# ChengZhang-98/lqer

Measured on AMD Instinct MI355X. Metric: W4A8+rank-r Linear GEMM TFLOPS-equiv, higher is better.
Workload: dtype bf16; 1 GPU; LqerLinear 4096x4096 rank32 W4A8-MXINT16 M=2048 (BASELINE configs[1]); rank=32, formats=x MXINT8/16, W MXINT4/16, A_out,B_out as x, y fp16, weights=one Linear

## Files before the change

include/lqer_hip.h:

```cpp
#ifndef LQER_HIP_H
#define LQER_HIP_H

#include <stddef.h>
#include <stdint.h>

#ifdef __cplusplus
extern "C" {
#endif

#define LQER_ABI_VERSION 14

#define LQER_OK 0
#define LQER_E_INVALID (-1)
#define LQER_E_UNSUPPORTED (-2)
#define LQER_E_LAUNCH (-3)
#define LQER_E_WORKSPACE (-4)

#define LQER_F32 0
#define LQER_F16 1
#define LQER_BF16 2

#define LQER_Q_PASSTHROUGH 0
#define LQER_Q_MXINT 1
#define LQER_Q_PASSTHROUGH_F16 2
// ... 16 lines not shown
  int32_t width;
  int32_t block;
  int32_t exp_width;
  int32_t exp_bias;
} lqer_qfmt_t;

typedef struct lqer_linear_desc {
  int32_t in_features;
  int32_t out_features;
  int32_t rank;
  int32_t has_bias;
  lqer_qfmt_t x_fmt;
  lqer_qfmt_t w_fmt;
  lqer_qfmt_t b_fmt;
  lqer_qfmt_t a_out_fmt;
  lqer_qfmt_t b_out_fmt;
  int32_t tuning;
} lqer_linear_desc_t;

#define LQER_TUNE_TILE_ROWS_128 0x1
#define LQER_TUNE_TILE_ROWS_64 0x2
#define LQER_TUNE_I8_ROWS_128 0x4
#define LQER_TUNE_I8_ROWS_256 0x8
#define LQER_TUNE_AMAX_ATOMIC 0x40000
#define LQER_TUNE_AMAX_PARTS 0x80000
#define LQER_TUNE_AMAX_XCH_MISS 0x100000
#define LQER_TUNE_ACT8_SPLIT 0x200000
#define LQER_TUNE_ACT8_FUSED 0x400000
#define LQER_TUNE_ACT16_SPLIT 0x800000
#define LQER_TUNE_ACT16_FUSED 0x1000000
#define LQER_TUNE_AMAX_NO_MRX 0x4000000
#define LQER_TUNE_BOUT_IN_PROLOGUE 0x2000000
#define LQER_TUNE_W_EXP_TABLE 0x8000000
#define LQER_TUNE_DECODE_NO_POLL 0x10000

typedef struct lqer_linear_sizes {
  size_t w_packed;
  size_t a_t;
  size_t b_t;
  size_t bias_q;
  size_t workspace;
} lqer_linear_sizes_t;

int lqer_version(void);
const char* lqer_last_error(void);
size_t lqer_sizeof_qfmt(void);
size_t lqer_sizeof_linear_desc(void);
size_t lqer_sizeof_linear_sizes(void);
size_t lqer_sizeof_group_member(void);

int64_t lqer_padded_k(int64_t K);
int64_t lqer_padded_n(int64_t N);
int64_t lqer_padded_m(int64_t M);
int64_t lqer_padded_r(int64_t r);


int lqer_quantize_mxint(const void* x, int dtype, int64_t rows, int64_t cols, int64_t ld,
                        const lqer_qfmt_t* fmt, float* deq_f32, int8_t* codes, int8_t* exps,
                        void* stream);

int lqer_quantize_mxint_tiles(const void* x, int dtype, int64_t batches, int64_t rows, int64_t cols, const lqer_qfmt_t* fmt,
                              int64_t tile_rows, int64_t tile_cols, float* deq_f32, float* amax_scratch, void* stream);

int lqer_quantize_act_mxint(const void* x, int dtype, int64_t M, int64_t K, int64_t ldx,
                            const lqer_qfmt_t* fmt, void* xq_bf16, void* stream);

// ... 193 lines not shown
```

lqer_amd/_lib.py:

```python
from __future__ import annotations

import ctypes as C
import os
import subprocess
from typing import Optional

_HERE = os.path.dirname(os.path.abspath(__file__))
LIB_PATH = os.environ.get("LQER_AMD_LIB") or os.path.join(_HERE, "liblqer_hip.so")
BUILD_SCRIPT = os.path.join(_HERE, "csrc", "build.sh")

ABI_VERSION = 14
F32, F16, BF16 = 0, 1, 2
Q_PASSTHROUGH, Q_MXINT, Q_PASSTHROUGH_F16, Q_MXINT_I8, Q_INT, Q_MINIFLOAT = 0, 1, 2, 3, 4, 5
K_ALIGN, M_ALIGN, N_ALIGN, R_ALIGN = 64, 256, 256, 16
ROUTE_SMALLM, ROUTE_TILE128, ROUTE_TILE256, ROUTE_I8 = 0, 1, 2, 3
TUNE_TILE_ROWS_128, TUNE_TILE_ROWS_64, TUNE_DECODE_NO_POLL = 0x1, 0x2, 0x10000
TUNE_I8_ROWS_128, TUNE_I8_ROWS_256, TUNE_AMAX_ATOMIC, TUNE_AMAX_PARTS = 0x4, 0x8, 0x40000, 0x80000
TUNE_ACT16_SPLIT, TUNE_ACT16_FUSED = 0x800000, 0x1000000
TUNE_ACT8_SPLIT, TUNE_ACT8_FUSED = 0x200000, 0x400000
TUNE_AMAX_NO_MRX = 0x4000000
TUNE_BOUT_IN_PROLOGUE = 0x2000000
TUNE_W_EXP_TABLE = 0x8000000
TUNE_AMAX_XCH_MISS = 0x100000


class QFmt(C.Structure):
    _fields_ = [("kind", C.c_int32), ("width", C.c_int32), ("block", C.c_int32), ("exp_width", C.c_int32), ("exp_bias", C.c_int32)]


class LinearDesc(C.Structure):
    _fields_ = [
        ("in_features", C.c_int32),
        ("out_features", C.c_int32),
        ("rank", C.c_int32),
        ("has_bias", C.c_int32),
        ("x_fmt", QFmt),
        ("w_fmt", QFmt),
        ("b_fmt", QFmt),
        ("a_out_fmt", QFmt),
        ("b_out_fmt", QFmt),
        ("tuning", C.c_int32),
    ]


class GroupMember(C.Structure):
    _fields_ = [("desc", C.POINTER(LinearDesc)), ("w_packed", C.c_void_p), ("b_t", C.c_void_p), ("b_limbs", C.c_int32),
                ("bias_q", C.c_void_p), ("y", C.c_void_p), ("ldy", C.c_int64)]


class LinearSizes(C.Structure):
    _fields_ = [("w_packed", C.c_size_t), ("a_t", C.c_size_t), ("b_t", C.c_size_t), ("bias_q", C.c_size_t), ("workspace", C.c_size_t)]


_vp, _i, _i64, _sz = C.c_void_p, C.c_int, C.c_int64, C.c_size_t
# ... 130 lines not shown
```

lqer_amd/csrc/gemm_plan.h:

```cpp
#pragma once
#include "common.h"

namespace lqer {

enum AmaxTravel {
  AMAX_NONE = 0,
  AMAX_CELLS,
  AMAX_PARTS,
  AMAX_XCH,
  AMAX_MRX,
};

struct GemmPlan {
  int err, launch_err;
  char msg[256];
  bool empty;

  int bout;
  int bout_L, bout_nblk;
  int route;
  int tile_rows;
  int tiles_m, tiles_n;
  unsigned grid;

  bool lowrank;
  bool f16x;
  bool staged, defer;
  bool w_twos, w_mf;
  bool i8_shift, i8_codes;
  int mt;

  AmaxTravel amax;
  size_t need;
  size_t zero_bytes;
  size_t prep_zero_bytes;
  struct {
    bool lds;
    int rg, nks;
    unsigned grid;
    int tiles_n32, seg_tiles;
    int nseg;
  } pre;
};

GemmPlan plan_gemm(const GemmArgs& shape, bool lowrank, bool i8_image, int dtype, int cus);

int device_cus();

int gemm_launch(const GemmPlan& p, GemmArgs g, int dtype, void* scratch, size_t scratch_bytes, bool amax_zeroed, hipStream_t st);
int launch_amax(const GemmPlan& p, const GemmArgs& g, bool amax_zeroed, hipStream_t st);
int tile128_launch(const GemmPlan& p, const GemmArgs& g, int dtype, hipStream_t st);
int m256_launch(const GemmPlan& p, const GemmArgs& g, int dtype, hipStream_t st);
int i8_launch(const GemmPlan& p, const GemmArgs& g, int dtype, hipStream_t st);
int smallm_launch(const GemmPlan& p, const GemmArgs& g, int dtype, hipStream_t st);

}
```

lqer_amd/csrc/gemm_plan.hip:

```cpp
#include <stdarg.h>
#include <stdio.h>

#include "gemm_plan.h"

namespace lqer {

namespace {

constexpr int64_t PLAN_CUS = 256;

int refuse(GemmPlan& p, bool at_launch, int code, const char* fmt, ...) {
  if (p.err || p.launch_err) return code;
  (at_launch ? p.launch_err : p.err) = code;
  va_list ap;
  va_start(ap, fmt);
  vsnprintf(p.msg, sizeof(p.msg), fmt, ap);
  va_end(ap);
  return code;
}

int64_t rounds(int64_t tiles) { return (tiles + PLAN_CUS - 1) / PLAN_CUS; }

int i8_tile_rows(const GemmArgs& g) {
  if (g.tuning & LQER_TUNE_I8_ROWS_128) return 128;
// ... 130 lines not shown
    if (p.amax == AMAX_CELLS || p.amax == AMAX_PARTS) plan_prepass(p, g);
  }

  if (i8_image && !i8_ok)
    refuse(p, true, LQER_E_UNSUPPORTED,
           "linear_gemm: LQER_Q_MXINT_I8 is not served for M=%d here (lqer_gemm_route != LQER_ROUTE_I8): call with LQER_Q_MXINT", g.M);
  switch (p.route) {
    case LQER_ROUTE_I8:
      p.tiles_m = (g.M + p.tile_rows - 1) / p.tile_rows, p.tiles_n = g.Np / BN;
      p.grid = (unsigned)(p.tiles_m * p.tiles_n < PLAN_CUS ? p.tiles_m * p.tiles_n : PLAN_CUS);
      p.i8_codes = g.w_i8codes, p.i8_shift = g.i8_shift;
      break;
    case LQER_ROUTE_SMALLM:
      p.grid = (unsigned)(g.Np / 16);
      p.mt = g.M > 48 ? 4 : (g.M + 15) / 16;
      break;
    case LQER_ROUTE_TILE256:
      p.tiles_m = (g.M + 255) / 256, p.tiles_n = g.Np / BN;
      p.grid = (unsigned)(p.tiles_m * p.tiles_n);
      break;
    default:
      p.tiles_m = (g.M + p.tile_rows - 1) / p.tile_rows, p.tiles_n = g.Np / BN;
      p.grid = (unsigned)(p.tiles_m * p.tiles_n);
      p.w_twos = g.w_twos, p.w_mf = g.w_mf;
      if (p.f16x && (p.w_mf || p.bout == 3))
        refuse(p, true, LQER_E_UNSUPPORTED,
               "linear_gemm: minifloat weights and B_out have no fp16 main loop (pass-through fp16 activations take the limb route)");
      else if (p.f16x && p.w_twos)
        refuse(p, true, LQER_E_UNSUPPORTED,
               "linear_gemm: integer weights have no fp16 main loop (pass-through fp16 activations take the limb route)");
      p.staged = lowrank && (p.w_twos || p.w_mf || g.rp * g.b_limbs > LQER_STAGE_MIN);
      p.defer = p.bout == 1 && !nibbles128 && p.tile_rows == 128 && !(g.tuning & LQER_TUNE_BOUT_IN_PROLOGUE) && g.Kp / BK >= 16 &&
                g.bout.kind == LQER_Q_MXINT && g.bout.mmax <= 4194304.0f && g.bout.mneg <= 4194304.0f && g.bout.tiny >= 1e-8f;
      break;
  }
  return p;
}

}
```

lqer_amd/csrc/gemm_w4a8.hip:

```cpp
#include <type_traits>
#include <utility>

#include "gemm_plan.h"
#include "gemm_tile.h"

namespace lqer {

#ifndef LQER_DEPTH
#define LQER_DEPTH 3
#endif
constexpr int DEPTH = LQER_DEPTH;
constexpr int NSLOT = DEPTH + 1;
constexpr int R_SLOT = (BN / 16) * LQER_PANEL_BYTES;
constexpr int OFF_A = 0;
constexpr int a_slot_bytes(int mt) { return 32 * mt * BK * 2; }
constexpr int gemm_lds_bytes(int mt) { return NSLOT * a_slot_bytes(mt) + NSLOT * R_SLOT; }

template <int OFF>
__device__ __forceinline__ bf16x8 lds_read128(uint32_t addr) {
  bf16x8 v;
  asm volatile("ds_read_b128 %0, %1 offset:%2" : "=v"(v) : "v"(addr), "i"(OFF));
  return v;
}
__device__ __forceinline__ u32x4 lds_read128u(uint32_t addr) {
  u32x4 v;
  asm volatile("ds_read_b128 %0, %1" : "=v"(v) : "v"(addr));
  return v;
}
__device__ __forceinline__ uint32_t lds_read32_512(uint32_t addr) {
  uint32_t v;
  asm volatile("ds_read_b32 %0, %1 offset:512" : "=v"(v) : "v"(addr));
  return v;
}
__device__ __forceinline__ u32x2 lds_read64(uint32_t addr) {
  u32x2 v;
  asm volatile("ds_read_b64 %0, %1" : "=v"(v) : "v"(addr));
  return v;
}
__device__ __forceinline__ int lds_read_i8_512(uint32_t addr) {
  int v;
  asm volatile("ds_read_i8 %0, %1 offset:512" : "=v"(v) : "v"(addr));
  return v;
}
__device__ __forceinline__ void lds_write128(uint32_t addr, u32x4 v) {
  asm volatile("ds_write_b128 %0, %1" ::"v"(addr), "v"(v) : "memory");
}
__device__ __forceinline__ void lds_wait(bf16x8& a, bf16x8& b, bf16x8& c, bf16x8& d) {
  asm volatile("s_waitcnt lgkmcnt(0)" : "+v"(a), "+v"(b), "+v"(c), "+v"(d));
}
__device__ __forceinline__ void lds_wait(bf16x8& a, bf16x8& b) {
  asm volatile("s_waitcnt lgkmcnt(0)" : "+v"(a), "+v"(b));
}
__device__ __forceinline__ void lds_wait(u32x2& a, int& b) {
  asm volatile("s_waitcnt lgkmcnt(0)" : "+v"(a), "+v"(b));
}

#ifdef LQER_STAMPS
#define LQER_LOAD_BARRIER ""
#else
#define LQER_LOAD_BARRIER "\n\ts_barrier"
#endif
#if defined(LQER_STAMPS) || defined(LQER_CLOCKPROBE)
__device__ unsigned long long* g_stamp_buf = nullptr;
#endif
#ifdef LQER_STAMPS
#define STAMP(i)                                                                        \
  do {                                                                                  \
    unsigned long long t_;                                                              \
    __builtin_amdgcn_sched_barrier(0);                                                  \
    asm volatile("s_memtime %0\n\ts_waitcnt lgkmcnt(0)" : "=s"(t_)::"memory");         \
    __builtin_amdgcn_sched_barrier(0);                                                  \
    st_sum[i] += t_ - st_prev;                                                          \
    st_prev = t_;                                                                       \
  } while (0)
#else
#define STAMP(i)
#endif

template <int DT, bool LOWRANK, int BOUT, bool STAGED = false, int MT = 4, bool WTWOS = false, bool DEFER = false, bool WMF = false>
__global__ __launch_bounds__(512) void k_lqer_gemm(GemmArgs g) {
  static_assert(MT == 4 || MT == 2, "128- or 64-row tiles");
  static_assert(!DEFER || (LOWRANK && BOUT == 1 && MT == 4), "deferred B_out: blocks of 16 on 128-row tiles");
  static_assert(!WTWOS || DT != LQER_F16X, "integer weights: no fp16 main loop");
  constexpr int BMk = 32 * MT;
  constexpr int AP = MT / 2;
  constexpr bool XF16 = DT == LQER_F16X;
  constexpr int A_SLOT = a_slot_bytes(MT), OFF_R = NSLOT * A_SLOT;
  extern __shared__ __attribute__((aligned(16))) unsigned char smem[];
  const int tid = threadIdx.x, lane = tid & 63;
  const int wave = __builtin_amdgcn_readfirstlane(tid >> 6);
  const int wn = wave;
  const int l31 = lane & 31, lh = lane >> 5;
#ifdef LQER_CLOCKPROBE
  unsigned long long cp_rin, cp_rq = 0;
  asm volatile("s_memrealtime %0\n\ts_waitcnt lgkmcnt(0)" : "=s"(cp_rin)::"memory");
#endif

  const int tile = xcd_tile(blockIdx.x, g.tiles_m * g.tiles_n);
  const int tm = tile / g.tiles_n, tn = tile - tm * g.tiles_n;
  const int m0 = tm * BMk, n0 = tn * BN;
  const int nk = g.Kp / BK;

  const auto a_rsrc = __builtin_amdgcn_make_buffer_rsrc((void*)(g.xq + (int64_t)m0 * g.Kp), 0, BMk * g.Kp * 2, 0x00020000);
  int a_voff[2] = {0, 0};
#pragma unroll
  for (int i = 0; i < AP; ++i) {
    const int row = wave * (8 * AP) + i * 8 + (lane >> 3);
    const int chunk = (lane & 7) ^ ((row >> 1) & 7);
    a_voff[i] = (row * g.Kp + chunk * 8) * 2;
  }
  const uint8_t* w_base = g.wp + ((int64_t)(n0 / 16) * nk) * LQER_PANEL_BYTES;
  const auto w_rsrc = __builtin_amdgcn_make_buffer_rsrc((void*)w_base, 0, 16 * nk * LQER_PANEL_BYTES, 0x00020000);
  const int w_voff = w_piece_voff(wave, lane, nk), w_voff8 = w_piece_voff(8, lane, nk);
  unsigned char* const a_dst0 = smem + OFF_A + wave * (8 * AP) * 128;
  unsigned char* const w_dst0 = smem + OFF_R + wave * 1024;
  auto issue_loads = [&](int kt, int slot) {
#pragma unroll
    for (int i = 0; i < AP; ++i)
      __builtin_amdgcn_raw_ptr_buffer_load_lds(a_rsrc, (lds_void*)(a_dst0 + slot * A_SLOT + i * 1024), 16, a_voff[i],
                                               kt * (BK * 2), 0, 0);
    __builtin_amdgcn_raw_ptr_buffer_load_lds(w_rsrc, (lds_void*)(w_dst0 + slot * R_SLOT), 16, w_voff, kt * LQER_PANEL_BYTES, 0, 0);
    if (wave == 0)
      __builtin_amdgcn_raw_ptr_buffer_load_lds(w_rsrc, (lds_void*)(smem + OFF_R + 8192 + slot * R_SLOT), 16, w_voff8,
                                               kt * LQER_PANEL_BYTES, 0, 0);
  };
  const uint32_t lds0 = (uint32_t)(uintptr_t)(lds_void*)smem;
  uint32_t fa_addr[4];
#pragma unroll
  for (int ks = 0; ks < 4; ++ks) fa_addr[ks] = lds0 + OFF_A + swz(l31, 2 * ks + lh);
  const int nw = wn * 32 + l31;
  const uint32_t fw_addr = lds0 + OFF_R + (nw >> 4) * LQER_PANEL_BYTES + (nw & 15) * 32 + lh * 16;
  const uint32_t fe_addr = lds0 + OFF_R + (nw >> 4) * LQER_PANEL_BYTES + (nw & 15) * 4;

  constexpr int STG = STAGED ? BMk * 8 / 512 : 1;
  u32x4 stg[STG];
  bf16x8 sb[STAGED ? 2 : 1][STAGED ? 4 : 1];
  const uint32_t stage = lds0 + OFF_A + (NSLOT - 1) * A_SLOT;
  const bf16_t* const bt_row = STAGED ? g.bt + (int64_t)(n0 + wn * 32 + l31) * g.rp + 8 * lh : nullptr;
  auto side_fetch_b = [&](int p0, int l, auto buf_c) {
    constexpr int BUF = decltype(buf_c)::value;
    if constexpr (STAGED) {
      const int cols = g.rp - p0 < 64 ? g.rp - p0 : 64;
#pragma unroll
      for (int ks = 0; ks < 4; ++ks)
        if (l < g.b_limbs && ks * 16 < cols) sb[BUF][ks] = *(const bf16x8*)(bt_row + (int64_t)l * g.Np * g.rp + p0 + ks * 16);
    }
  };
  auto side_fetch = [&](int p0) {
    if constexpr (!STAGED) return;
    const int cols = g.rp - p0 < 64 ? g.rp - p0 : 64;
    const int cpr = cols >> 3;
#pragma unroll
    for (int j = 0; j < STG; ++j) {
      const int c = tid + 512 * j;
      if (c < BMk * cpr) {
        const int row = c / cpr, ch = c - row * cpr;
        stg[j] = *(const u32x4*)(g.xaq + (int64_t)(m0 + row) * g.xaq_ld + p0 + 8 * ch);
      }
    }
    side_fetch_b(p0, 0, std::integral_constant<int, 0>{});
  };
  constexpr bool side_staged = LOWRANK && STAGED;
  if constexpr (side_staged) side_fetch(0);
  constexpr bool side_direct = LOWRANK && !STAGED;
  bf16x8 db[side_direct ? 2 : 1], dx[side_direct ? 2 : 1][side_direct ? MT : 1];
  const bool two_limbs = g.b_limbs > 1;
  if constexpr (side_direct) {
#pragma unroll
    for (int sl = 0; sl < 2; ++sl) {
      const int l = two_limbs ? sl : 0, ks = two_limbs ? 0 : sl;
      if (l < g.b_limbs && ks * 16 < g.rp) {
        db[sl] = *(const bf16x8*)(g.bt + ((int64_t)l * g.Np + n0 + wn * 32 + l31) * g.rp + ks * 16 + 8 * lh);
#pragma unroll
        for (int i = 0; i < MT; ++i) dx[sl][i] = *(const bf16x8*)(g.xaq + (int64_t)(m0 + i * 32 + l31) * g.xaq_ld + ks * 16 + 8 * lh);
      }
    }
  }

#pragma unroll
  for (int d = 0; d < DEPTH; ++d) issue_loads(d, d);

  f32x16 acc[MT];
#pragma unroll
  for (int i = 0; i < MT; ++i)
#pragma unroll
    for (int k = 0; k < 16; ++k) acc[i][k] = 0.f;
  f32x16 sp[DEFER ? MT : 1];
  if constexpr (DEFER) {
#pragma unroll
    for (int i = 0; i < MT; ++i)
#pragma unroll
      for (int k = 0; k < 16; ++k) sp[i][k] = 0.f;
  }
  auto side_acc = [&](int i) -> f32x16& {
    if constexpr (DEFER) return sp[i];
    else return acc[i];
  };

  if constexpr (LOWRANK) {
    if constexpr (side_direct) {
#pragma unroll
      for (int sl = 0; sl < 2; ++sl) {
        const int l = two_limbs ? sl : 0, ks = two_limbs ? 0 : sl;
        if (l < g.b_limbs && ks * 16 < g.rp) {
#pragma unroll
          for (int i = 0; i < MT; ++i) side_acc(i) = __builtin_amdgcn_mfma_f32_32x32x16_bf16(db[sl], dx[sl][i], side_acc(i), 0, 0, 0);
        }
      }
    }
    if constexpr (side_staged)
    for (int p0 = 0; p0 < g.rp; p0 += 64) {
      const int cols = g.rp - p0 < 64 ? g.rp - p0 : 64;
      const int cpr = cols >> 3;
      if (p0) {
        asm volatile("s_barrier" ::: "memory");
        side_fetch(p0);
      }
#pragma unroll
      for (int j = 0; j < STG; ++j) {
        const int c = tid + 512 * j;
        if (c < BMk * cpr) {
          const int row = c / cpr, ch = c - row * cpr;
          lds_write128(stage + swz(row, ch), stg[j]);
        }
      }
      asm volatile("s_waitcnt lgkmcnt(0)\n\ts_barrier" ::: "memory");
      auto limb = [&](int l, auto buf_c) {
        constexpr int BUF = decltype(buf_c)::value;
        if (l >= g.b_limbs) return;
        side_fetch_b(p0, l + 1, std::integral_constant<int, BUF ^ 1>{});
#pragma unroll
        for (int ks = 0; ks < 4; ++ks)
          if (ks * 16 < cols) {
            const uint32_t fa = stage + swz(l31, 2 * ks + lh);
            if constexpr (MT == 4) {
              bf16x8 x0 = lds_read128<0>(fa), x1 = lds_read128<4096>(fa), x2 = lds_read128<8192>(fa), x3 = lds_read128<12288>(fa);
              lds_wait(x0, x1, x2, x3);
              side_acc(0) = __builtin_amdgcn_mfma_f32_32x32x16_bf16(sb[BUF][ks], x0, side_acc(0), 0, 0, 0);
              side_acc(1) = __builtin_amdgcn_mfma_f32_32x32x16_bf16(sb[BUF][ks], x1, side_acc(1), 0, 0, 0);
// ... 23 lines not shown
#pragma unroll
      for (int i = 0; i < MT; ++i)
#pragma unroll
        for (int b = 0; b < 2; ++b) {
          float amax;
          if constexpr (BOUT == 1) {
            amax = 0.f;
#pragma unroll
            for (int k = 0; k < 8; ++k) amax = fmaxf(amax, fabsf(acc[i][8 * b + k]));
            amax = pair32_max(amax);
          } else {
            amax = g.bout_amax ? g.bout_amax[(int64_t)(m0 + i * 32 + l31) * g.bout_nblk + (n0 + wn * 32 + 16 * b) / g.bout_L] : 1.0f;
          }
          const int e = block_exponent(amax, g.bout);
          float blk[8];
#pragma unroll
          for (int k = 0; k < 8; ++k) blk[k] = acc[i][8 * b + k];
          mxint_requant_fast(blk, e, g.bout);
#pragma unroll
          for (int k = 0; k < 8; ++k) acc[i][8 * b + k] = blk[k];
        }
    }
  }
  if (g.bias) {
#pragma unroll
    for (int k = 0; k < 16; ++k) {
      const float bv = g.bias[acc_col(n0 + wn * 32, k, lh)];
#pragma unroll
      for (int i = 0; i < MT; ++i) acc[i][k] += bv;
    }
  }

  const bool late = wave >= 4;
  if constexpr (MT == 4) asm volatile("s_waitcnt vmcnt(6)\n\ts_barrier" ::: "memory");
  else asm volatile("s_waitcnt vmcnt(4)\n\ts_barrier" ::: "memory");
  if (late) asm volatile("s_barrier" ::: "memory");
#ifdef LQER_CLOCKPROBE
  unsigned long long cp_c0, cp_r0;
  asm volatile("s_memtime %0\n\ts_memrealtime %1\n\ts_waitcnt lgkmcnt(0)" : "=s"(cp_c0), "=s"(cp_r0)::"memory");
#endif
#ifdef LQER_STAMPS
  unsigned long long st_sum[8] = {0, 0, 0, 0, 0, 0, 0, 0}, st_prev;
  asm volatile("s_memtime %0\n\ts_waitcnt lgkmcnt(0)" : "=s"(st_prev)::"memory");
#endif
  const u32x2 a_rs01 = ring_rsrc_base(g.xq + (int64_t)m0 * g.Kp);
  const u32x4 a_rs = {a_rs01[0], a_rs01[1], (uint32_t)(BMk * g.Kp * 2), 0x00020000u};
  const u32x2 w_rs01 = ring_rsrc_base(w_base);
  const u32x4 w_rs = {w_rs01[0], w_rs01[1], (uint32_t)(16 * nk * LQER_PANEL_BYTES), 0x00020000u};
  const uint32_t m0_a = lds0 + OFF_A + wave * (8 * AP) * 128;
  const uint32_t m0_w = lds0 + OFF_R + wave * 1024;
  const uint32_t m0_w8 = lds0 + OFF_R + 8192;
  float dq_s = 1.f, dq_inv = 1.f;
  auto defer_piece = [&](auto piece_c) {
    constexpr int P = decltype(piece_c)::value;
    if constexpr (DEFER && P >= 0) {
      typedef __attribute__((ext_vector_type(2))) float f2;
      constexpr int J = P >> 1, I = J >> 1, B8 = 8 * (J & 1);
      if constexpr ((P & 1) == 0) {
        float amax = 0.f;
#pragma unroll
        for (int k = 0; k < 8; k += 2) amax = fmaxf(fmaxf(amax, fabsf(sp[I][B8 + k])), fabsf(sp[I][B8 + k + 1]));
        amax = pair32_max(amax);
        int up = g.bout.mbits - block_exponent(amax, g.bout);
        up = up > 126 ? 126 : (up < -126 ? -126 : up);
        dq_s = __uint_as_float((uint32_t)(127 + up) << 23);
        dq_inv = __uint_as_float((uint32_t)(127 - up) << 23);
      } else {
        const float es = g.bout.eps * dq_s, hi = g.bout.mmax, lo = -g.bout.mneg, tiny = g.bout.tiny;
        const f2 magic = {12582912.0f, 12582912.0f};
#pragma unroll
        for (int k = 0; k < 8; k += 2) {
          const f2 x = {sp[I][B8 + k], sp[I][B8 + k + 1]};
          const f2 c = {copysignf(es, x[0]), copysignf(es, x[1])};
          f2 r = (__builtin_elementwise_fma(x, (f2){dq_s, dq_s}, c) + magic) - magic;
          r[0] = __builtin_amdgcn_fmed3f(r[0], lo, hi);
          r[1] = __builtin_amdgcn_fmed3f(r[1], lo, hi);
          const f2 val = r * (f2){dq_inv, dq_inv};
          sp[I][B8 + k] = fabsf(x[0]) <= tiny ? x[0] : val[0];
          sp[I][B8 + k + 1] = fabsf(x[1]) <= tiny ? x[1] : val[1];
        }
      }
    }
  };
  auto defer_pin = [&](auto piece_c) {
    constexpr int P = decltype(piece_c)::value;
    (void)dq_s, (void)dq_inv, (void)sp;
    if constexpr (DEFER && P >= 0) {
      constexpr int J = P >> 1, I = J >> 1, B8 = 8 * (J & 1);
      if constexpr ((P & 1) == 0) asm volatile("" : "+v"(dq_s), "+v"(dq_inv));
      else
        asm volatile("" : "+v"(sp[I][B8]), "+v"(sp[I][B8 + 1]), "+v"(sp[I][B8 + 2]), "+v"(sp[I][B8 + 3]), "+v"(sp[I][B8 + 4]), "+v"(sp[I][B8 + 5]),
                     "+v"(sp[I][B8 + 6]), "+v"(sp[I][B8 + 7]));
    }
  };
  auto step = [&](int kt, auto slot_c, auto piece_c) {
    constexpr int SLOT = decltype(slot_c)::value;
    constexpr int slot_new = SLOT == 0 ? NSLOT - 1 : SLOT - 1;
    STAMP(7);
    __builtin_amdgcn_s_setprio(1);
    const int ktn = __builtin_amdgcn_readfirstlane(kt + DEPTH);
    const int a_soff = ktn * (BK * 2), w_soff = ktn * LQER_PANEL_BYTES;
    const uint32_t m0a0 = m0_a + slot_new * A_SLOT, m0a1 = m0a0 + 1024;
    const uint32_t m0w = m0_w + slot_new * R_SLOT, m0w8 = m0_w8 + slot_new * R_SLOT;
    bf16x8 xa[4][MT];
    u32x4 wr;
    uint32_t we;
    if constexpr (MT == 4) {
      asm volatile(
          "ds_read_b128 %0, %18 offset:%c25\n\tds_read_b32 %1, %19 offset:%c25+512\n\t"
          LQER_READ_X2("%2", "%3", "%20", "%c24") LQER_READ_X2("%4", "%5", "%20", "%c24+8192")
          LQER_READ_X2("%6", "%7", "%21", "%c24") LQER_READ_X2("%8", "%9", "%21", "%c24+8192")
          LQER_READ_X2("%10", "%11", "%22", "%c24") LQER_READ_X2("%12", "%13", "%22", "%c24+8192")
          LQER_READ_X2("%14", "%15", "%23", "%c24") LQER_READ_X2("%16", "%17", "%23", "%c24+8192")
          LQER_LDS_DMA("%32", "%26", "%30", "%36") LQER_LDS_DMA("%33", "%27", "%30", "%36") LQER_LDS_DMA("%34", "%28", "%31", "%37")
          "s_cmp_lg_u32 %38, 0\n\ts_cbranch_scc1 1f\n\t"
          LQER_LDS_DMA("%35", "%29", "%31", "%37")
          "1:\n\ts_waitcnt vmcnt(6) lgkmcnt(0)"
          : "=&v"(wr), "=&v"(we), "=&v"(xa[0][0]), "=&v"(xa[0][1]), "=&v"(xa[0][2]), "=&v"(xa[0][3]), "=&v"(xa[1][0]),
            "=&v"(xa[1][1]), "=&v"(xa[1][2]), "=&v"(xa[1][3]), "=&v"(xa[2][0]), "=&v"(xa[2][1]), "=&v"(xa[2][2]),
            "=&v"(xa[2][3]), "=&v"(xa[3][0]), "=&v"(xa[3][1]), "=&v"(xa[3][2]), "=&v"(xa[3][3])
          : "v"(fw_addr), "v"(fe_addr), "v"(fa_addr[0]), "v"(fa_addr[1]), "v"(fa_addr[2]), "v"(fa_addr[3]),
            "i"(SLOT * A_SLOT), "i"(SLOT * R_SLOT),
            "v"(a_voff[0]), "v"(a_voff[1]), "v"(w_voff), "v"(w_voff8),
            "s"(a_rs), "s"(w_rs), "s"(m0a0), "s"(m0a1), "s"(m0w), "s"(m0w8), "s"(a_soff), "s"(w_soff), "s"(wave)
          : "memory", "scc");
    } else {
      asm volatile(
          "ds_read_b128 %0, %10 offset:%c17\n\tds_read_b32 %1, %11 offset:%c17+512\n\t"
          LQER_READ_X2("%2", "%3", "%12", "%c16") LQER_READ_X2("%4", "%5", "%13", "%c16")
          LQER_READ_X2("%6", "%7", "%14", "%c16") LQER_READ_X2("%8", "%9", "%15", "%c16")
          LQER_LDS_DMA("%23", "%18", "%21", "%26") LQER_LDS_DMA("%24", "%19", "%22", "%27")
          "s_cmp_lg_u32 %28, 0\n\ts_cbranch_scc1 1f\n\t"
          LQER_LDS_DMA("%25", "%20", "%22", "%27")
          "1:\n\ts_waitcnt vmcnt(4) lgkmcnt(0)"
          : "=&v"(wr), "=&v"(we), "=&v"(xa[0][0]), "=&v"(xa[0][1]), "=&v"(xa[1][0]), "=&v"(xa[1][1]), "=&v"(xa[2][0]),
            "=&v"(xa[2][1]), "=&v"(xa[3][0]), "=&v"(xa[3][1])
          : "v"(fw_addr), "v"(fe_addr), "v"(fa_addr[0]), "v"(fa_addr[1]), "v"(fa_addr[2]), "v"(fa_addr[3]),
            "i"(SLOT * A_SLOT), "i"(SLOT * R_SLOT),
            "v"(a_voff[0]), "v"(w_voff), "v"(w_voff8),
            "s"(a_rs), "s"(w_rs), "s"(m0a0), "s"(m0w), "s"(m0w8), "s"(a_soff), "s"(w_soff), "s"(wave)
          : "memory", "scc");
    }
    STAMP(1);
    constexpr bool WLIN = !WMF && !WTWOS && !XF16;
    if constexpr (WLIN) we += 0x09090909u;
    auto expand = [&](uint32_t word, uint32_t scale_bits) {
      if constexpr (WMF) return expand_frag_lut(word, scale_bits, g.w_lut[0], g.w_lut[1]);
      else if constexpr (WTWOS) return expand_frag_twos(word, scale_bits);
      else if constexpr (WLIN) return expand_frag_lin(word, scale_bits);
      else return expand_frag_t<XF16>(word, scale_bits);
    };
    bf16x8 wb_first = expand(wr[0], exp_byte_bits<0>(we));
    asm volatile("s_barrier" : "+v"(wb_first)::"memory");
    __builtin_amdgcn_s_setprio(0);
    __builtin_amdgcn_sched_barrier(0);
    STAMP(4);
    defer_piece(piece_c);
    const uint32_t sc[4] = {0u, exp_byte_bits<1>(we), exp_byte_bits<2>(we), exp_byte_bits<3>(we)};
#pragma unroll
    for (int ks = 0; ks < 4; ++ks) {
      const bf16x8 wb = ks == 0 ? wb_first : expand(wr[ks], sc[ks]);
#pragma unroll
      for (int i = 0; i < MT; ++i) acc[i] = mfma_32x32x16<XF16>(wb, xa[ks][i], acc[i]);
    }
    defer_pin(piece_c);
    __builtin_amdgcn_sched_barrier(0);
    STAMP(5);
    asm volatile("s_barrier" ::: "memory");
    __builtin_amdgcn_sched_barrier(0);
    STAMP(6);
  };
  using std::integral_constant;
  constexpr integral_constant<int, -1> no_piece{};
  int kt0 = 0;
  if constexpr (DEFER) {
#define LQER_DSTEP(KT) step(KT, integral_constant<int, (KT) % NSLOT>{}, integral_constant<int, KT>{})
    LQER_DSTEP(0); LQER_DSTEP(1); LQER_DSTEP(2); LQER_DSTEP(3); LQER_DSTEP(4); LQER_DSTEP(5); LQER_DSTEP(6); LQER_DSTEP(7);
    LQER_DSTEP(8); LQER_DSTEP(9); LQER_DSTEP(10); LQER_DSTEP(11); LQER_DSTEP(12); LQER_DSTEP(13); LQER_DSTEP(14); LQER_DSTEP(15);
#undef LQER_DSTEP
    kt0 = 16;
  }
  if (kt0 < nk)
  for (int kt = kt0;; kt += NSLOT) {
    step(kt, integral_constant<int, 0>{}, no_piece);
    if (kt + 1 >= nk) break;
    step(kt + 1, integral_constant<int, 1>{}, no_piece);
    if (kt + 2 >= nk) break;
    step(kt + 2, integral_constant<int, 2>{}, no_piece);
    if (kt + 3 >= nk) break;
    step(kt + 3, integral_constant<int, 3>{}, no_piece);
    if (kt + 4 >= nk) break;
  }
  asm volatile("s_waitcnt vmcnt(0)" ::: "memory");
  if (!late) asm volatile("s_barrier" ::: "memory");
#ifdef LQER_CLOCKPROBE
  {
    unsigned long long cp_c1, cp_r1;
    asm volatile("s_memtime %0\n\ts_memrealtime %1\n\ts_waitcnt lgkmcnt(0)" : "=s"(cp_c1), "=s"(cp_r1)::"memory");
    if (g_stamp_buf && lane == 0) {
      g_stamp_buf[(blockIdx.x * 8 + wave) * 8 + 0] = cp_c1 - cp_c0;
      g_stamp_buf[(blockIdx.x * 8 + wave) * 8 + 1] = cp_r1 - cp_r0;
      g_stamp_buf[(blockIdx.x * 8 + wave) * 8 + 2] = cp_rin;
      g_stamp_buf[(blockIdx.x * 8 + wave) * 8 + 3] = cp_r0;
      g_stamp_buf[(blockIdx.x * 8 + wave) * 8 + 4] = cp_r1;
      g_stamp_buf[(blockIdx.x * 8 + wave) * 8 + 7] = cp_rq;
    }
  }
#endif
#ifdef LQER_STAMPS
  if (g_stamp_buf && lane == 0)
    for (int i = 0; i < 8; ++i) g_stamp_buf[(blockIdx.x * 8 + wave) * 8 + i] = st_sum[i];
#endif

  if constexpr (DEFER) {
#pragma unroll
    for (int i = 0; i < MT; ++i)
#pragma unroll
      for (int k = 0; k < 16; ++k) acc[i][k] += sp[i][k];
  }
  const bool aligned16 = (((uintptr_t)g.y) & 15) == 0;
  const int nb = n0 + wn * 32;
#pragma unroll
  for (int i = 0; i < MT; ++i) {
    const int m = m0 + i * 32 + l31;
    if constexpr (DT == LQER_F32) {
#pragma unroll
      for (int q = 0; q < 4; ++q) {
        const int n = nb + 8 * q + 4 * lh;
        if (m < g.M) {
          float* dst = (float*)g.y + (int64_t)m * g.ldy + n;
          if (n + 3 < g.N && (g.ldy & 3) == 0 && aligned16) {
            *(float4*)dst = make_float4(acc[i][4 * q], acc[i][4 * q + 1], acc[i][4 * q + 2], acc[i][4 * q + 3]);
          } else {
#pragma unroll
            for (int t = 0; t < 4; ++t)
              if (n + t < g.N) dst[t] = acc[i][4 * q + t];
          }
        }
      }
    } else {
      uint32_t pk[4][2];
#pragma unroll
      for (int q = 0; q < 4; ++q)
#pragma unroll
        for (int h = 0; h < 2; ++h) {
          const float v0 = acc[i][4 * q + 2 * h], v1 = acc[i][4 * q + 2 * h + 1];
          if constexpr (DT == LQER_F16 || DT == LQER_F16X) {
            typedef __attribute__((ext_vector_type(2))) _Float16 h2;
            h2 hv = {(_Float16)v0, (_Float16)v1};
            pk[q][h] = __builtin_bit_cast(uint32_t, hv);
          } else {
            pk[q][h] = (uint32_t)f32_to_bf16_rne(v0) | ((uint32_t)f32_to_bf16_rne(v1) << 16);
          }
        }
      const bool wide = (g.ldy & 7) == 0 && nb + 32 <= g.N && aligned16;
#pragma unroll
// ... 4 lines not shown
          auto r1 = __builtin_amdgcn_permlane32_swap(a1, b1, false, false);
          if (m < g.M) {
            bf16_t* dst = (bf16_t*)g.y + (int64_t)m * g.ldy + nb + 16 * p + 8 * lh;
            *(uint4*)dst = make_uint4(r0[0], r1[0], r0[1], r1[1]);
          }
        } else if (m < g.M) {
#pragma unroll
          for (int qq = 0; qq < 2; ++qq) {
            const int n = nb + 8 * (2 * p + qq) + 4 * lh;
            const uint32_t lo = qq ? b0 : a0, hi = qq ? b1 : a1;
            bf16_t* dst = (bf16_t*)g.y + (int64_t)m * g.ldy + n;
            if (n < g.N) dst[0] = (bf16_t)(lo & 0xffff);
            if (n + 1 < g.N) dst[1] = (bf16_t)(lo >> 16);
            if (n + 2 < g.N) dst[2] = (bf16_t)(hi & 0xffff);
            if (n + 3 < g.N) dst[3] = (bf16_t)(hi >> 16);
          }
        }
      }
    }
  }
#ifdef LQER_CLOCKPROBE
  {
    unsigned long long cp_r2, cp_r3;
    asm volatile("s_memrealtime %0\n\ts_waitcnt lgkmcnt(0)" : "=s"(cp_r2)::"memory");
    asm volatile("s_waitcnt vmcnt(0)\n\ts_memrealtime %0\n\ts_waitcnt lgkmcnt(0)" : "=s"(cp_r3)::"memory");
    if (g_stamp_buf && lane == 0) {
      g_stamp_buf[(blockIdx.x * 8 + wave) * 8 + 5] = cp_r2;
      g_stamp_buf[(blockIdx.x * 8 + wave) * 8 + 6] = cp_r3;
    }
  }
#endif
}

template <int DT, bool LR, int BO, bool ST, int MT, bool WTWOS, bool DEFER, bool WMF>
constexpr bool tile_variant_exists() {
  constexpr bool nibbles = WTWOS || WMF;
  if (WTWOS && WMF) return false;
  if ((nibbles || BO == 3) && (MT != 4 || DT == LQER_F16X)) return false;
  if (!LR) return BO == 0 && !ST && !DEFER;
  if (nibbles) return ST && !DEFER;
  if (DEFER) return BO == 1 && MT == 4;
  return true;
}

template <int DT, int I>
static bool run_tile(int key, const GemmPlan& p, const GemmArgs& g, hipStream_t st, int& rc) {
  constexpr bool LR = I & 1, ST = I & 2, WTWOS = I & 8, DEFER = I & 16, WMF = I & 32;
  constexpr int MT = I & 4 ? 2 : 4, BO = I >> 6;
  if constexpr (tile_variant_exists<DT, LR, BO, ST, MT, WTWOS, DEFER, WMF>()) {
    if (key == I) {
      rc = launch_k<k_lqer_gemm<DT, LR, BO, ST, MT, WTWOS, DEFER, WMF>>("lqer_gemm", p.grid, 512, gemm_lds_bytes(MT), st, g);
      return true;
    }
  }
  return false;
}

template <int DT, int... I>
static int launch_tile(const GemmPlan& p, const GemmArgs& g, hipStream_t st, std::integer_sequence<int, I...>) {
  const int key = p.lowrank | p.staged << 1 | (p.tile_rows == 64) << 2 | p.w_twos << 3 | p.defer << 4 | p.w_mf << 5 | p.bout << 6;
  int rc;
  if ((run_tile<DT, I>(key, p, g, st, rc) || ...)) return rc;
  set_error("linear_gemm: the plan asks for a tile kernel variant that does not exist (%#x)", key);
  return LQER_E_UNSUPPORTED;
}

int tile128_launch(const GemmPlan& p, const GemmArgs& g, int dtype, hipStream_t st) {
  constexpr std::make_integer_sequence<int, 4 << 6> variants{};
  return with_dtype(dtype, [&](auto dt) {
    constexpr int DT = decltype(dt)::value;
    if constexpr (DT == LQER_F16)
      if (p.f16x) return launch_tile<LQER_F16X>(p, g, st, variants);
    return launch_tile<DT>(p, g, st, variants);
  });
}

#if defined(LQER_STAMPS) || defined(LQER_CLOCKPROBE)
extern "C" int lqer_debug_set_stamp_buffer(void* p) {
  return (int)hipMemcpyToSymbol(HIP_SYMBOL(g_stamp_buf), &p, sizeof(p));
}
#endif

}
```

Before: 1087 TFLOP/s-equiv.

## Split K across wave halves in deferred B_out tile kernel with LDS reduction

```diff
diff --git a/include/lqer_hip.h b/include/lqer_hip.h
--- a/include/lqer_hip.h
+++ b/include/lqer_hip.h
@@ -72,6 +72,7 @@
 #define LQER_TUNE_AMAX_NO_MRX 0x4000000
 #define LQER_TUNE_BOUT_IN_PROLOGUE 0x2000000
 #define LQER_TUNE_W_EXP_TABLE 0x8000000
+#define LQER_TUNE_NO_KSPLIT 0x10000000
 #define LQER_TUNE_DECODE_NO_POLL 0x10000
 
 typedef struct lqer_linear_sizes {
diff --git a/lqer_amd/_lib.py b/lqer_amd/_lib.py
--- a/lqer_amd/_lib.py
+++ b/lqer_amd/_lib.py
@@ -20,6 +20,7 @@
 TUNE_ACT8_SPLIT, TUNE_ACT8_FUSED = 0x200000, 0x400000
 TUNE_AMAX_NO_MRX = 0x4000000
 TUNE_BOUT_IN_PROLOGUE = 0x2000000
+TUNE_NO_KSPLIT = 0x10000000
 TUNE_W_EXP_TABLE = 0x8000000
 TUNE_AMAX_XCH_MISS = 0x100000
 
diff --git a/lqer_amd/csrc/gemm_plan.h b/lqer_amd/csrc/gemm_plan.h
--- a/lqer_amd/csrc/gemm_plan.h
+++ b/lqer_amd/csrc/gemm_plan.h
@@ -26,6 +26,7 @@
   bool lowrank;
   bool f16x;
   bool staged, defer;
+  bool ksplit;
   bool w_twos, w_mf;
   bool i8_shift, i8_codes;
   int mt;
diff --git a/lqer_amd/csrc/gemm_plan.hip b/lqer_amd/csrc/gemm_plan.hip
--- a/lqer_amd/csrc/gemm_plan.hip
+++ b/lqer_amd/csrc/gemm_plan.hip
@@ -186,6 +186,7 @@
       p.staged = lowrank && (p.w_twos || p.w_mf || g.rp * g.b_limbs > LQER_STAGE_MIN);
       p.defer = p.bout == 1 && !nibbles128 && p.tile_rows == 128 && !(g.tuning & LQER_TUNE_BOUT_IN_PROLOGUE) && g.Kp / BK >= 16 &&
                 g.bout.kind == LQER_Q_MXINT && g.bout.mmax <= 4194304.0f && g.bout.mneg <= 4194304.0f && g.bout.tiny >= 1e-8f;
+      p.ksplit = p.defer && !p.staged && !p.f16x && !(g.tuning & LQER_TUNE_NO_KSPLIT);
       break;
   }
   return p;
diff --git a/lqer_amd/csrc/gemm_w4a8.hip b/lqer_amd/csrc/gemm_w4a8.hip
--- a/lqer_amd/csrc/gemm_w4a8.hip
+++ b/lqer_amd/csrc/gemm_w4a8.hip
@@ -15,6 +15,8 @@
 constexpr int OFF_A = 0;
 constexpr int a_slot_bytes(int mt) { return 32 * mt * BK * 2; }
 constexpr int gemm_lds_bytes(int mt) { return NSLOT * a_slot_bytes(mt) + NSLOT * R_SLOT; }
+constexpr int KS_STASH_B = 4096, KS_STASH_BYTES = KS_STASH_B + 8 * 2048, KS_XCH = 8192;
+static_assert(8 * KS_XCH <= gemm_lds_bytes(4), "the exchange lies inside the ring");
 
 template <int OFF>
 __device__ __forceinline__ bf16x8 lds_read128(uint32_t addr) {
@@ -44,6 +46,10 @@
 }
 __device__ __forceinline__ void lds_write128(uint32_t addr, u32x4 v) {
   asm volatile("ds_write_b128 %0, %1" ::"v"(addr), "v"(v) : "memory");
+}
+template <int OFF>
+__device__ __forceinline__ void lds_write128_at(uint32_t addr, f32x4 v) {
+  asm volatile("ds_write_b128 %0, %1 offset:%2" ::"v"(addr), "v"(v), "i"(OFF) : "memory");
 }
 __device__ __forceinline__ void lds_wait(bf16x8& a, bf16x8& b, bf16x8& c, bf16x8& d) {
   asm volatile("s_waitcnt lgkmcnt(0)" : "+v"(a), "+v"(b), "+v"(c), "+v"(d));
@@ -77,11 +83,12 @@
 #define STAMP(i)
 #endif
 
-template <int DT, bool LOWRANK, int BOUT, bool STAGED = false, int MT = 4, bool WTWOS = false, bool DEFER = false, bool WMF = false>
-__global__ __launch_bounds__(512) void k_lqer_gemm(GemmArgs g) {
+template <int DT, bool LOWRANK, int BOUT, bool STAGED, int MT, bool WTWOS, bool DEFER, bool WMF, bool KSPLIT>
+__device__ __forceinline__ void gemm_tile_body(const GemmArgs& g) {
   static_assert(MT == 4 || MT == 2, "128- or 64-row tiles");
   static_assert(!DEFER || (LOWRANK && BOUT == 1 && MT == 4), "deferred B_out: blocks of 16 on 128-row tiles");
   static_assert(!WTWOS || DT != LQER_F16X, "integer weights: no fp16 main loop");
+  static_assert(!KSPLIT || (DEFER && !STAGED && !WTWOS && !WMF && DT != LQER_F16X), "k split: deferred B_out, direct side path, plain nibbles, bf16");
   constexpr int BMk = 32 * MT;
   constexpr int AP = MT / 2;
   constexpr bool XF16 = DT == LQER_F16X;
@@ -89,7 +96,8 @@
   extern __shared__ __attribute__((aligned(16))) unsigned char smem[];
   const int tid = threadIdx.x, lane = tid & 63;
   const int wave = __builtin_amdgcn_readfirstlane(tid >> 6);
-  const int wn = wave;
+  const int kh = KSPLIT ? wave >> 2 : 0;
+  const int wn = KSPLIT ? 2 * (wave & 3) + kh : wave;
   const int l31 = lane & 31, lh = lane >> 5;
 #ifdef LQER_CLOCKPROBE
   unsigned long long cp_rin, cp_rq = 0;
@@ -125,12 +133,20 @@
                                                kt * LQER_PANEL_BYTES, 0, 0);
   };
   const uint32_t lds0 = (uint32_t)(uintptr_t)(lds_void*)smem;
+  uint32_t stash0 = 0;
+  if constexpr (KSPLIT) {
+    __shared__ __attribute__((aligned(16))) unsigned char ks_stash[KS_STASH_BYTES];
+    stash0 = (uint32_t)(uintptr_t)(lds_void*)ks_stash;
+  }
   uint32_t fa_addr[4];
 #pragma unroll
-  for (int ks = 0; ks < 4; ++ks) fa_addr[ks] = lds0 + OFF_A + swz(l31, 2 * ks + lh);
+  for (int ks = 0; ks < 4; ++ks) fa_addr[ks] = lds0 + OFF_A + swz(l31, 2 * (KSPLIT ? (2 * kh + ks) & 3 : ks) + lh);
   const int nw = wn * 32 + l31;
   const uint32_t fw_addr = lds0 + OFF_R + (nw >> 4) * LQER_PANEL_BYTES + (nw & 15) * 32 + lh * 16;
   const uint32_t fe_addr = lds0 + OFF_R + (nw >> 4) * LQER_PANEL_BYTES + (nw & 15) * 4;
+  const uint32_t ks_fw = fw_addr + 8 * kh, ks_fe = fe_addr + 2 * kh;
+  const uint32_t ks_fw_o = kh ? ks_fw - 2 * LQER_PANEL_BYTES : ks_fw + 2 * LQER_PANEL_BYTES;
+  const uint32_t ks_fe_o = kh ? ks_fe - 2 * LQER_PANEL_BYTES : ks_fe + 2 * LQER_PANEL_BYTES;
 
   constexpr int STG = STAGED ? BMk * 8 / 512 : 1;
   u32x4 stg[STG];
@@ -169,6 +185,10 @@
 #pragma unroll
     for (int sl = 0; sl < 2; ++sl) {
       const int l = two_limbs ? sl : 0, ks = two_limbs ? 0 : sl;
+      if constexpr (KSPLIT) {
+        db[sl] = bf16x8{};
+        dx[sl][2] = dx[sl][3] = bf16x8{};
+      }
       if (l < g.b_limbs && ks * 16 < g.rp) {
         db[sl] = *(const bf16x8*)(g.bt + ((int64_t)l * g.Np + n0 + wn * 32 + l31) * g.rp + ks * 16 + 8 * lh);
 #pragma unroll
@@ -185,12 +205,20 @@
   for (int i = 0; i < MT; ++i)
 #pragma unroll
     for (int k = 0; k < 16; ++k) acc[i][k] = 0.f;
-  f32x16 sp[DEFER ? MT : 1];
+  constexpr int SPT = KSPLIT ? 2 : MT;
+  f32x16 sp[DEFER ? SPT : 1];
   if constexpr (DEFER) {
 #pragma unroll
+    for (int i = 0; i < SPT; ++i)
+#pragma unroll
+      for (int k = 0; k < 16; ++k) sp[i][k] = 0.f;
+  }
+  f32x16 acc_o[KSPLIT ? MT : 1];
+  if constexpr (KSPLIT) {
+#pragma unroll
     for (int i = 0; i < MT; ++i)
 #pragma unroll
-      for (int k = 0; k < 16; ++k) sp[i][k] = 0.f;
+      for (int k = 0; k < 16; ++k) acc_o[i][k] = 0.f;
   }
   auto side_acc = [&](int i) -> f32x16& {
     if constexpr (DEFER) return sp[i];
@@ -204,7 +232,18 @@
         const int l = two_limbs ? sl : 0, ks = two_limbs ? 0 : sl;
         if (l < g.b_limbs && ks * 16 < g.rp) {
 #pragma unroll
-          for (int i = 0; i < MT; ++i) side_acc(i) = __builtin_amdgcn_mfma_f32_32x32x16_bf16(db[sl], dx[sl][i], side_acc(i), 0, 0, 0);
+          for (int i = 0; i < SPT; ++i) side_acc(i) = __builtin_amdgcn_mfma_f32_32x32x16_bf16(db[sl], dx[sl][i], side_acc(i), 0, 0, 0);
+        }
+      }
+      if constexpr (KSPLIT) {
+        const uint32_t st_b = stash0 + KS_STASH_B + wave * 2048 + lane * 16, st_x = stash0 + lane * 16;
+#pragma unroll
+        for (int sl = 0; sl < 2; ++sl) {
+          lds_write128(st_b + sl * 1024, __builtin_bit_cast(u32x4, db[sl]));
+          if (wave == 0) {
+            lds_write128(st_x + (2 * sl) * 1024, __builtin_bit_cast(u32x4, dx[sl][2]));
+            lds_write128(st_x + (2 * sl + 1) * 1024, __builtin_bit_cast(u32x4, dx[sl][3]));
+          }
         }
       }
     }
@@ -294,7 +333,8 @@
   }
 
   const bool late = wave >= 4;
-  if constexpr (MT == 4) asm volatile("s_waitcnt vmcnt(6)\n\ts_barrier" ::: "memory");
+  if constexpr (KSPLIT) asm volatile("s_waitcnt vmcnt(6) lgkmcnt(0)\n\ts_barrier" ::: "memory");
+  else if constexpr (MT == 4) asm volatile("s_waitcnt vmcnt(6)\n\ts_barrier" ::: "memory");
   else asm volatile("s_waitcnt vmcnt(4)\n\ts_barrier" ::: "memory");
   if (late) asm volatile("s_barrier" ::: "memory");
 #ifdef LQER_CLOCKPROBE
@@ -317,7 +357,7 @@
     constexpr int P = decltype(piece_c)::value;
     if constexpr (DEFER && P >= 0) {
       typedef __attribute__((ext_vector_type(2))) float f2;
-      constexpr int J = P >> 1, I = J >> 1, B8 = 8 * (J & 1);
+      constexpr int J = P >> 1, I = (J >> 1) % SPT, B8 = 8 * (J & 1);
       if constexpr ((P & 1) == 0) {
         float amax = 0.f;
 #pragma unroll
@@ -348,7 +388,7 @@
     constexpr int P = decltype(piece_c)::value;
     (void)dq_s, (void)dq_inv, (void)sp;
     if constexpr (DEFER && P >= 0) {
-      constexpr int J = P >> 1, I = J >> 1, B8 = 8 * (J & 1);
+      constexpr int J = P >> 1, I = (J >> 1) % SPT, B8 = 8 * (J & 1);
       if constexpr ((P & 1) == 0) asm volatile("" : "+v"(dq_s), "+v"(dq_inv));
       else
         asm volatile("" : "+v"(sp[I][B8]), "+v"(sp[I][B8 + 1]), "+v"(sp[I][B8 + 2]), "+v"(sp[I][B8 + 3]), "+v"(sp[I][B8 + 4]), "+v"(sp[I][B8 + 5]),
@@ -367,7 +407,40 @@
     bf16x8 xa[4][MT];
     u32x4 wr;
     uint32_t we;
-    if constexpr (MT == 4) {
+    constexpr int P = decltype(piece_c)::value;
+    u32x2 wr2[2];
+    uint32_t we2[2];
+    bf16x8 sdb[2], sdx[2][2];
+    if constexpr (KSPLIT) {
+      if constexpr (P == 8) {
+        const uint32_t st_b = stash0 + KS_STASH_B + wave * 2048 + lane * 16, st_x = stash0 + lane * 16;
+        asm volatile(
+            "ds_read_b128 %0, %6\n\tds_read_b128 %1, %6 offset:1024\n\t"
+            "ds_read_b128 %2, %7\n\tds_read_b128 %3, %7 offset:1024\n\tds_read_b128 %4, %7 offset:2048\n\tds_read_b128 %5, %7 offset:3072\n\t"
+            "s_waitcnt lgkmcnt(0)"
+            : "=&v"(sdb[0]), "=&v"(sdb[1]), "=&v"(sdx[0][0]), "=&v"(sdx[0][1]), "=&v"(sdx[1][0]), "=&v"(sdx[1][1])
+            : "v"(st_b), "v"(st_x)
+            : "memory");
+      }
+      asm volatile(
+          "ds_read_b64 %[w0], %[fw] offset:%c[ro]\n\tds_read_b64 %[w1], %[fwo] offset:%c[ro]\n\t"
+          "ds_read_u16 %[e0], %[fe] offset:%c[ro]+512\n\tds_read_u16 %[e1], %[feo] offset:%c[ro]+512\n\t"
+          LQER_READ_X2("%[x00]", "%[x01]", "%[fa0]", "%c[ao]") LQER_READ_X2("%[x02]", "%[x03]", "%[fa0]", "%c[ao]+8192")
+          LQER_READ_X2("%[x10]", "%[x11]", "%[fa1]", "%c[ao]") LQER_READ_X2("%[x12]", "%[x13]", "%[fa1]", "%c[ao]+8192")
+          LQER_LDS_DMA("%[ma0]", "%[av0]", "%[ars]", "%[aso]") LQER_LDS_DMA("%[ma1]", "%[av1]", "%[ars]", "%[aso]")
+          LQER_LDS_DMA("%[mw]", "%[wv]", "%[wrs]", "%[wso]")
+          "s_cmp_lg_u32 %[wv0], 0\n\ts_cbranch_scc1 1f\n\t"
+          LQER_LDS_DMA("%[mw8]", "%[wv8]", "%[wrs]", "%[wso]")
+          "1:\n\ts_waitcnt vmcnt(6) lgkmcnt(0)"
+          : [w0] "=&v"(wr2[0]), [w1] "=&v"(wr2[1]), [e0] "=&v"(we2[0]), [e1] "=&v"(we2[1]), [x00] "=&v"(xa[0][0]), [x01] "=&v"(xa[0][1]),
+            [x02] "=&v"(xa[0][2]), [x03] "=&v"(xa[0][3]), [x10] "=&v"(xa[1][0]), [x11] "=&v"(xa[1][1]), [x12] "=&v"(xa[1][2]),
+            [x13] "=&v"(xa[1][3])
+          : [fw] "v"(ks_fw), [fwo] "v"(ks_fw_o), [fe] "v"(ks_fe), [feo] "v"(ks_fe_o), [fa0] "v"(fa_addr[0]), [fa1] "v"(fa_addr[1]),
+            [ao] "i"(SLOT * A_SLOT), [ro] "i"(SLOT * R_SLOT), [av0] "v"(a_voff[0]), [av1] "v"(a_voff[1]), [wv] "v"(w_voff),
+            [wv8] "v"(w_voff8), [ars] "s"(a_rs), [wrs] "s"(w_rs), [ma0] "s"(m0a0), [ma1] "s"(m0a1), [mw] "s"(m0w), [mw8] "s"(m0w8),
+            [aso] "s"(a_soff), [wso] "s"(w_soff), [wv0] "s"(wave)
+          : "memory", "scc");
+    } else if constexpr (MT == 4) {
       asm volatile(
           "ds_read_b128 %0, %18 offset:%c25\n\tds_read_b32 %1, %19 offset:%c25+512\n\t"
           LQER_READ_X2("%2", "%3", "%20", "%c24") LQER_READ_X2("%4", "%5", "%20", "%c24+8192")
@@ -405,25 +478,60 @@
     }
     STAMP(1);
     constexpr bool WLIN = !WMF && !WTWOS && !XF16;
-    if constexpr (WLIN) we += 0x09090909u;
+    if constexpr (WLIN && !KSPLIT) we += 0x09090909u;
     auto expand = [&](uint32_t word, uint32_t scale_bits) {
       if constexpr (WMF) return expand_frag_lut(word, scale_bits, g.w_lut[0], g.w_lut[1]);
       else if constexpr (WTWOS) return expand_frag_twos(word, scale_bits);
       else if constexpr (WLIN) return expand_frag_lin(word, scale_bits);
       else return expand_frag_t<XF16>(word, scale_bits);
     };
+    if constexpr (KSPLIT) {
+      we2[0] += 0x0909u, we2[1] += 0x0909u;
+      wr[0] = wr2[0][0], we = we2[0];
+    }
     bf16x8 wb_first = expand(wr[0], exp_byte_bits<0>(we));
     asm volatile("s_barrier" : "+v"(wb_first)::"memory");
     __builtin_amdgcn_s_setprio(0);
     __builtin_amdgcn_sched_barrier(0);
     STAMP(4);
+    if constexpr (KSPLIT && P == 8) {
+#pragma unroll
+      for (int i = 0; i < 2; ++i) {
+#pragma unroll
+        for (int k = 0; k < 16; ++k) acc[i][k] += sp[i][k], sp[i][k] = 0.f;
+#pragma unroll
+        for (int sl = 0; sl < 2; ++sl) sp[i] = __builtin_amdgcn_mfma_f32_32x32x16_bf16(sdb[sl], sdx[sl][i], sp[i], 0, 0, 0);
+      }
+    }
     defer_piece(piece_c);
-    const uint32_t sc[4] = {0u, exp_byte_bits<1>(we), exp_byte_bits<2>(we), exp_byte_bits<3>(we)};
-#pragma unroll
-    for (int ks = 0; ks < 4; ++ks) {
-      const bf16x8 wb = ks == 0 ? wb_first : expand(wr[ks], sc[ks]);
-#pragma unroll
-      for (int i = 0; i < MT; ++i) acc[i] = mfma_32x32x16<XF16>(wb, xa[ks][i], acc[i]);
+    if constexpr (KSPLIT) {
+      const uint32_t sc[2][2] = {{0u, exp_byte_bits<1>(we2[0])}, {exp_byte_bits<0>(we2[1]), exp_byte_bits<1>(we2[1])}};
+#pragma unroll
+      for (int j = 0; j < 2; ++j)
+#pragma unroll
+        for (int h = 0; h < 2; ++h) {
+          const bf16x8 wb = j + h == 0 ? wb_first : expand(wr2[h][j], sc[h][j]);
+#pragma unroll
+          for (int i = 0; i < MT; ++i) {
+            if (h) acc_o[i] = mfma_32x32x16<XF16>(wb, xa[j][i], acc_o[i]);
+            else acc[i] = mfma_32x32x16<XF16>(wb, xa[j][i], acc[i]);
+          }
+        }
+      if constexpr (P < 0) {
+#pragma unroll
+        for (int n = 0; n < 16; ++n) {
+          __builtin_amdgcn_sched_group_barrier(0x008, 1, 0);
+          __builtin_amdgcn_sched_group_barrier(0x002, 3, 0);
+        }
+      }
+    } else {
+      const uint32_t sc[4] = {0u, exp_byte_bits<1>(we), exp_byte_bits<2>(we), exp_byte_bits<3>(we)};
+#pragma unroll
+      for (int ks = 0; ks < 4; ++ks) {
+        const bf16x8 wb = ks == 0 ? wb_first : expand(wr[ks], sc[ks]);
+#pragma unroll
+        for (int i = 0; i < MT; ++i) acc[i] = mfma_32x32x16<XF16>(wb, xa[ks][i], acc[i]);
+      }
     }
     defer_pin(piece_c);
     __builtin_amdgcn_sched_barrier(0);
@@ -476,14 +584,44 @@
 
   if constexpr (DEFER) {
 #pragma unroll
-    for (int i = 0; i < MT; ++i)
-#pragma unroll
-      for (int k = 0; k < 16; ++k) acc[i][k] += sp[i][k];
-  }
+    for (int i = 0; i < SPT; ++i)
+#pragma unroll
+      for (int k = 0; k < 16; ++k) acc[MT - SPT + i][k] += sp[i][k];
+  }
+  if constexpr (KSPLIT) {
+    asm volatile("s_barrier" ::: "memory");
+  }
+  auto add_partner = [&](int i) {
+    if constexpr (KSPLIT) {
+      if (i == 0 || i == 2) {
+        const uint32_t x_out = lds0 + wave * KS_XCH + lane * 16;
+        if (i == 2) asm volatile("s_barrier" ::: "memory");
+#pragma unroll
+        for (int j = 0; j < 2; ++j) {
+          lds_write128_at<0>(x_out + j * 4096, __builtin_shufflevector(acc_o[i + j], acc_o[i + j], 0, 1, 2, 3));
+          lds_write128_at<1024>(x_out + j * 4096, __builtin_shufflevector(acc_o[i + j], acc_o[i + j], 4, 5, 6, 7));
+          lds_write128_at<2048>(x_out + j * 4096, __builtin_shufflevector(acc_o[i + j], acc_o[i + j], 8, 9, 10, 11));
+          lds_write128_at<3072>(x_out + j * 4096, __builtin_shufflevector(acc_o[i + j], acc_o[i + j], 12, 13, 14, 15));
+        }
+        asm volatile("s_waitcnt lgkmcnt(0)\n\ts_barrier" ::: "memory");
+      }
+      const uint32_t x_in = lds0 + (wave ^ 4) * KS_XCH + lane * 16 + (i & 1) * 4096;
+      f32x4 q0, q1, q2, q3;
+      asm volatile(
+          "ds_read_b128 %0, %4\n\tds_read_b128 %1, %4 offset:1024\n\tds_read_b128 %2, %4 offset:2048\n\t"
+          "ds_read_b128 %3, %4 offset:3072\n\ts_waitcnt lgkmcnt(0)"
+          : "=&v"(q0), "=&v"(q1), "=&v"(q2), "=&v"(q3)
+          : "v"(x_in)
+          : "memory");
+#pragma unroll
+      for (int t = 0; t < 4; ++t) acc[i][t] += q0[t], acc[i][4 + t] += q1[t], acc[i][8 + t] += q2[t], acc[i][12 + t] += q3[t];
+    }
+  };
   const bool aligned16 = (((uintptr_t)g.y) & 15) == 0;
   const int nb = n0 + wn * 32;
 #pragma unroll
   for (int i = 0; i < MT; ++i) {
+    add_partner(i);
     const int m = m0 + i * 32 + l31;
     if constexpr (DT == LQER_F32) {
 #pragma unroll
@@ -554,10 +692,21 @@
 #endif
 }
 
-template <int DT, bool LR, int BO, bool ST, int MT, bool WTWOS, bool DEFER, bool WMF>
+template <int DT, bool LOWRANK, int BOUT, bool STAGED = false, int MT = 4, bool WTWOS = false, bool DEFER = false, bool WMF = false>
+__global__ __launch_bounds__(512) void k_lqer_gemm(GemmArgs g) {
+  constexpr bool KSPLIT = DEFER && !STAGED && !WTWOS && !WMF && DT != LQER_F16X;
+  gemm_tile_body<DT, LOWRANK, BOUT, STAGED, MT, WTWOS, DEFER, WMF, KSPLIT>(g);
+}
+template <int DT>
+__global__ __launch_bounds__(512) void k_lqer_gemm_nks(GemmArgs g) {
+  gemm_tile_body<DT, true, 1, false, 4, false, true, false, false>(g);
+}
+
+template <int DT, bool LR, int BO, bool ST, int MT, bool WTWOS, bool DEFER, bool WMF, bool NKS>
 constexpr bool tile_variant_exists() {
   constexpr bool nibbles = WTWOS || WMF;
   if (WTWOS && WMF) return false;
+  if (NKS && !(LR && BO == 1 && DEFER && !ST && MT == 4 && !nibbles && DT != LQER_F16X)) return false;
   if ((nibbles || BO == 3) && (MT != 4 || DT == LQER_F16X)) return false;
   if (!LR) return BO == 0 && !ST && !DEFER;
   if (nibbles) return ST && !DEFER;
@@ -568,10 +717,12 @@
 template <int DT, int I>
 static bool run_tile(int key, const GemmPlan& p, const GemmArgs& g, hipStream_t st, int& rc) {
   constexpr bool LR = I & 1, ST = I & 2, WTWOS = I & 8, DEFER = I & 16, WMF = I & 32;
-  constexpr int MT = I & 4 ? 2 : 4, BO = I >> 6;
-  if constexpr (tile_variant_exists<DT, LR, BO, ST, MT, WTWOS, DEFER, WMF>()) {
+  constexpr bool NKS = I & 256;
+  constexpr int MT = I & 4 ? 2 : 4, BO = (I >> 6) & 3;
+  if constexpr (tile_variant_exists<DT, LR, BO, ST, MT, WTWOS, DEFER, WMF, NKS>()) {
     if (key == I) {
-      rc = launch_k<k_lqer_gemm<DT, LR, BO, ST, MT, WTWOS, DEFER, WMF>>("lqer_gemm", p.grid, 512, gemm_lds_bytes(MT), st, g);
+      if constexpr (NKS) rc = launch_k<k_lqer_gemm_nks<DT>>("lqer_gemm", p.grid, 512, gemm_lds_bytes(MT), st, g);
+      else rc = launch_k<k_lqer_gemm<DT, LR, BO, ST, MT, WTWOS, DEFER, WMF>>("lqer_gemm", p.grid, 512, gemm_lds_bytes(MT), st, g);
       return true;
     }
   }
@@ -580,7 +731,8 @@
 
 template <int DT, int... I>
 static int launch_tile(const GemmPlan& p, const GemmArgs& g, hipStream_t st, std::integer_sequence<int, I...>) {
-  const int key = p.lowrank | p.staged << 1 | (p.tile_rows == 64) << 2 | p.w_twos << 3 | p.defer << 4 | p.w_mf << 5 | p.bout << 6;
+  const int key = p.lowrank | p.staged << 1 | (p.tile_rows == 64) << 2 | p.w_twos << 3 | p.defer << 4 | p.w_mf << 5 | p.bout << 6 |
+                  (p.defer && !p.staged && !p.f16x && !p.ksplit) << 8;
   int rc;
   if ((run_tile<DT, I>(key, p, g, st, rc) || ...)) return rc;
   set_error("linear_gemm: the plan asks for a tile kernel variant that does not exist (%#x)", key);
@@ -588,7 +740,7 @@
 }
 
 int tile128_launch(const GemmPlan& p, const GemmArgs& g, int dtype, hipStream_t st) {
-  constexpr std::make_integer_sequence<int, 4 << 6> variants{};
+  constexpr std::make_integer_sequence<int, 8 << 6> variants{};
   return with_dtype(dtype, [&](auto dt) {
     constexpr int DT = decltype(dt)::value;
     if constexpr (DT == LQER_F16)
```

Measured after the change: 1114 TFLOP/s-equiv (median of 6 runs). 2.5% higher.
